# xiph/theora

Measured on AMD Instinct MI355X. Metric: decode frames/sec (4k 4:2:0, bit-exact), higher is better.
Workload: dtype i16; 1 GPU; 4k (3840x2160 coded) 4:2:0, 4 concurrent streams per GPU, keyframe interval 64, content class 'dense', levels form (seeded fragment command streams resident in HBM), loop filter on (flimit 2); streams_per_gpu=4, frame_pool=6, gt_IC=True, parallelism=stream-sharded x1

## Files before the change

theora_amd/csrc/thip_decode.hip:

```cpp
#include <hip/hip_runtime.h>
#include <stdint.h>
#include <stdio.h>
#include <stdlib.h>
#include <string.h>
#include <time.h>

#include <atomic>
#include <mutex>
#include <vector>

#include "../../include/theora_hip.h"
#include "thip_device.h"
#include "thip_ctx.h"
#include "thip_device_guard.h"

using namespace thip;

#define HIP_TRY(expr)                                                                    \
  do {                                                                                   \
    hipError_t e_ = (expr);                                                              \
    if (e_ != hipSuccess) {                                                              \
      fprintf(stderr, "theora_hip: %s failed: %s (%s:%d)\n", #expr, hipGetErrorString(e_), \
              __FILE__, __LINE__);                                                       \
      return THIP_EFAULT;                                                                \
// ... 154 lines not shown
  int64_t frame_serial, out_serial;
  hipEvent_t ev_out2[2];
  int held_img;
  int64_t held_serial;
  int32_t *enq_last_lane;
  int enq_ncoded, enq_nuncoded, enq_nslots, enq_frame_type, enq_flimit, enq_active, enq_last_tile;
  int enq_lf_y0[3], enq_lf_y1[3], enq_lf_any;
  FrameExtras extras;
  int16_t *d_dc;
  uint4 *d_dc_ent;
  uint8_t *d_dc_rowhas;
  uint32_t *fault;
  struct {
    int valid;
    thip_frame_desc d;
    int ring[3];
    FrameExtras extras;
    int64_t serial;
    uint32_t launch_id;
  } redo;
  int redo_owned;
  uint8_t *d_edge;
  uint32_t edge_epoch;
  uint8_t *d_edge_sb;
  uint32_t edge_epoch_sb;
  int device_dc, enq_device_dc;
  int16_t *h_dc, *d_dc_in;
  uint8_t *h_flags, *d_flags;
  uint32_t *h_tok, *d_tok;
  uint32_t *h_slot_tok, *d_slot_tok;
  uint16_t *h_dq, *d_dq;
  uint16_t *h_dqp, *d_dqp;
  size_t tok_cap;
  int tok_ready;
  int enq_ntok, enq_tok_slots, enq_dense_slots;
  int enq_levels_hint;
  int enq_level_slots;
  int enq_tile_blocks;
  uint32_t *h_tl, *d_tl;
  uint32_t *h_tl_buf[2];
  int tl_buf;
  int64_t tl_buf_serial[2];
  size_t tl_cap;
  int tl_ready;
  int16_t *d_tl_tmp;
  uint8_t *d_tl_last;
// ... 381 lines not shown
  DeviceGuard dg(st->device);
  (void)hipDeviceSynchronize();
  if (st->fault) (void)hipHostFree(st->fault);
  for (int b = 0; b < 3; b++)
    if (st->frames[b]) (void)hipFree(st->frames[b]);
  if (st->coded_map) (void)hipFree(st->coded_map);
  if (st->h_info) (void)hipHostFree(st->h_info);
  if (st->h_coeffs) (void)hipHostFree(st->h_coeffs);
  if (st->h_slot0) (void)hipHostFree(st->h_slot0);
  for (int b = 0; b < 2; b++)
    if (st->h_out[b]) (void)hipHostFree(st->h_out[b]);
  for (int k = 0; k < 2; k++)
    if (st->ev_out2[k]) (void)hipEventDestroy(st->ev_out2[k]);
  if (st->ev_staging) (void)hipEventDestroy(st->ev_staging);
  if (st->d_info) (void)hipFree(st->d_info);
  if (st->d_coeffs) (void)hipFree(st->d_coeffs);
  if (st->d_slot0) (void)hipFree(st->d_slot0);
  if (st->d_dc) (void)hipFree(st->d_dc);
  if (st->d_dc_ent) (void)hipFree(st->d_dc_ent);
  if (st->d_dc_rowhas) (void)hipFree(st->d_dc_rowhas);
  if (st->ev_order) (void)hipEventDestroy(st->ev_order);
  if (st->d_edge) (void)hipFree(st->d_edge);
  if (st->d_edge_sb) (void)hipFree(st->d_edge_sb);
  for (int k = 0; k < 2; k++)
    if (st->h_tl_buf[k]) (void)hipHostFree(st->h_tl_buf[k]);
  if (st->d_tl) (void)hipFree(st->d_tl);
  if (st->d_tl_tmp) (void)hipFree(st->d_tl_tmp);
  if (st->d_tl_last) (void)hipFree(st->d_tl_last);
  if (st->d_tl_slot) (void)hipFree(st->d_tl_slot);
  if (st->d_tl_arr) (void)hipFree(st->d_tl_arr);
  if (st->d_tl_pos) (void)hipFree(st->d_tl_pos);
  if (st->d_tl_wide) (void)hipFree(st->d_tl_wide);
  if (st->d_tl_rank) (void)hipFree(st->d_tl_rank);
  if (st->d_frag_pos) (void)hipFree(st->d_frag_pos);
  if (st->pp_frame) (void)hipFree(st->pp_frame);
  if (st->pp_var) (void)hipFree(st->pp_var);
  if (st->pp_qis) (void)hipFree(st->pp_qis);
  if (st->pp_done) (void)hipFree(st->pp_done);
  if (st->h_pp_qis) (void)hipHostFree(st->h_pp_qis);
  if (st->ev_pp) (void)hipEventDestroy(st->ev_pp);
  if (st->d_dc_in) (void)hipFree(st->d_dc_in);
  if (st->h_dc) (void)hipHostFree(st->h_dc);
  if (st->h_flags) (void)hipHostFree(st->h_flags);
  if (st->h_tok) (void)hipHostFree(st->h_tok);
  if (st->h_slot_tok) (void)hipHostFree(st->h_slot_tok);
  if (st->h_dq) (void)hipHostFree(st->h_dq);
// ... 500 lines not shown
  if (fits && !dc_global) {
    HIP_TRY(set_dynamic_lds(reinterpret_cast<const void *>(k_dc_wave), kDcwLdsMax, 3));
    hipLaunchKernelGGL(k_dc_prepare, dim3(max_rows, 3, ndc), dim3((max_nh + 63) & ~63), 0, s, D);
    hipLaunchKernelGGL(k_dc_wave, dim3(3, ndc), dim3(64), (size_t)lds, s, D);
  } else {
    hipLaunchKernelGGL(k_dc_unpredict, dim3(3, ndc), dim3((max_rows + 63) & ~63), 0, s, D);
  }
  HIP_TRY(hipGetLastError());
  return THIP_OK;
}

static int take_edge_records(thip_state *st, StreamK &K, uint8_t **buf, uint32_t *epoch, size_t bytes, uint32_t tag, hipStream_t s) {
  if (!*buf) {
    HIP_TRY(hipMalloc((void **)buf, bytes));
    HIP_TRY(hipMemsetAsync(*buf, 0, bytes, s));
  }
  K.edge = *buf;
  *epoch = *epoch % 4095u + 1u;
  K.epoch = *epoch;
  st->redo.launch_id = K.epoch | tag;
  return THIP_OK;
}

static int launch_recon(Chunk &C, thip_state *const *states, bool levels, bool two_passes, hipStream_t s) {
  const BatchK &B = C.B;
  const int nlive = C.nlive;
  const int fuse = two_passes ? 0 : THIP_OPT("fuse");
  if (fuse == 3 && C.any_lf && !C.any_skip && xcd_round_robin(states[C.live[0]]->device)) {
    int longest = 1, total_tiles = 0;
    for (int j = 0; j < nlive; j++) total_tiles += B.s[j].tile_end[2];
    const int sb_tiles = THIP_OPT("sb_tiles");
    const bool small = sb_tiles > 0 && total_tiles < sb_tiles;
    for (int j = 0; j < nlive; j++) {
      thip_state *st = states[C.live[j]];
      StreamK &K = C.B.s[j];
      if (st->tiles.tiles_y[0] > 4096) return THIP_EIMPL;
      longest = std::max(longest, fill_bands(K, st));
      const int rc = small ? take_edge_records(st, K, &st->d_edge_sb, &st->edge_epoch_sb, (size_t)4 * K.tile_end[2] * Tf4::kRec, 0x1000u, s)
                           : take_edge_records(st, K, &st->d_edge, &st->edge_epoch, (size_t)K.tile_end[2] * kTfRec, 0u, s);
      if (rc < 0) return rc;
    }
    ScopedTimer t(s, THIP_KERNEL_RECON);
    if (small) {
      if (levels) hipLaunchKernelGGL(k_recon_lf_sb<true>, dim3(8 * longest, nlive), dim3(256), 0, s, B);
      else hipLaunchKernelGGL(k_recon_lf_sb<false>, dim3(8 * longest, nlive), dim3(256), 0, s, B);
    } else if (levels) hipLaunchKernelGGL(k_recon_lf<true>, dim3(8 * longest, nlive), dim3(64), 0, s, B);
    else hipLaunchKernelGGL(k_recon_lf<false>, dim3(8 * longest, nlive), dim3(64), 0, s, B);
  } else {
    {
      ScopedTimer t(s, THIP_KERNEL_RECON);
      if (levels) hipLaunchKernelGGL(k_recon<true>, dim3(C.max_wg, nlive), dim3(64 * THIP_RECON_WG_WAVES), 0, s, B);
      else hipLaunchKernelGGL(k_recon<false>, dim3(C.max_wg, nlive), dim3(64 * THIP_RECON_WG_WAVES), 0, s, B);
    }
    if (C.any_lf) {
      ScopedTimer t(s, THIP_KERNEL_LOOPFILTER);
      hipLaunchKernelGGL(k_loopfilter, dim3(C.max_seam_wg, nlive), dim3(THIP_LF_WG), 0, s, B);
    }
  }
  HIP_TRY(hipGetLastError());
  return THIP_OK;
}

static int advance_rings(const Chunk &C, thip_state *const *states, const thip_frame_desc *descs, hipStream_t s) {
// ... 1527 lines not shown
```

theora_amd/csrc/thip_fused.h:

```cpp
#pragma once

#ifndef THIP_TF_PITCH
#define THIP_TF_PITCH 144
#endif
template <int BW>
struct TfGeom {
  static constexpr int kBW = BW;
  static constexpr int kPitch = BW == 16 ? THIP_TF_PITCH : 8 * BW + 16;
  static constexpr int kX0 = 8;
  static constexpr int kImgRows = 40;
  static constexpr int kFlagOff = kImgRows * kPitch;
  static constexpr int kFlagPitch = BW + 4;
  static constexpr int kRowDwords = 2 * BW;
  static constexpr int kBotUnits = (2 * kRowDwords + 2) / 3, kRightUnits = 11;
  static constexpr int kBot = 0;
  static constexpr int kRight = kBotUnits * 16;
  static constexpr int kTop = (kBotUnits + kRightUnits) * 16;
  static constexpr int kRec = ((2 * kBotUnits + kRightUnits) * 16 + 127) & ~127;
};
typedef TfGeom<16> Tf16;
constexpr int kTfPitch = Tf16::kPitch, kTfX0 = Tf16::kX0, kTfImgRows = Tf16::kImgRows, kTfFlagOff = Tf16::kFlagOff, kTfFlagPitch = Tf16::kFlagPitch;
constexpr int kTfLds = 7168;
static_assert(kTfFlagOff + 6 * kTfFlagPitch <= kTfLds, "the image lives in the wave's staging area");
static_assert(kLdsTabOff + 768 <= kTfLds && kLdsTabOff >= 6 * 1024, "the tables sit behind six staged pieces");
constexpr int kTfUnit = 16;
constexpr int kTfBotUnits = Tf16::kBotUnits, kTfRightUnits = Tf16::kRightUnits;
constexpr int kTfBot = Tf16::kBot, kTfRight = Tf16::kRight, kTfTop = Tf16::kTop, kTfRec = Tf16::kRec;
static_assert(kTfBotUnits == 22 && kTfRight == 352 && kTfTop == 528 && kTfRec == 896, "the record layout of rounds 3 and 4");

typedef uint32_t tf_u32x4 __attribute__((ext_vector_type(4)));
__device__ __forceinline__ void tf_store_unit(uint8_t *p, uint4 v, bool through) {
  if (through) {
    const tf_u32x4 w = {v.x, v.y, v.z, v.w};
    asm volatile("global_store_dwordx4 %0, %1, off sc0 sc1" ::"v"(p), "v"(w) : "memory");
  } else {
    *reinterpret_cast<uint4 *>(p) = v;
  }
}
__device__ __forceinline__ uint4 tf_load_unit(const uint8_t *p) {
  tf_u32x4 w;
  asm volatile("global_load_dwordx4 %0, %1, off sc0 sc1\n\ts_waitcnt vmcnt(0)" : "=&v"(w) : "v"(p) : "memory");
  return make_uint4(w.x, w.y, w.z, w.w);
}

template <class G>
__device__ __forceinline__ int tf_rows_at(int idx, int ri0) { return (ri0 + idx / G::kRowDwords) * G::kPitch + G::kX0 + (idx % G::kRowDwords) * 4; }
template <class G>
// ... 188 lines not shown
#ifdef THIP_PRIO_SEQ
#define THIP_PRIO_AT(i) __builtin_amdgcn_s_setprio((THIP_PRIO_SEQ >> (12 - 4 * (i))) & 3)
#else
#define THIP_PRIO_AT(i) do { } while (0)
#endif
#ifndef THIP_TF_WAVES_PER_EU
#define THIP_TF_WAVES_PER_EU 5
#endif
template <bool LEVELS>
__global__ __launch_bounds__(64, THIP_TF_WAVES_PER_EU) void k_recon_lf(const BatchK B) {
  __shared__ uint4 s_tf[kTfLds / 16];
  const StreamK &S = B.s[blockIdx.y];
  const int lane = (int)threadIdx.x & 63;
  const int band = (int)blockIdx.x & 7, jb = (int)blockIdx.x >> 3;
  const uint2 *info_p = S.info;
  const int4 *coeffs_p = S.coeffs;
  const uint32_t *slot0_p = S.tile_slot0;
  uint8_t *self = S.self;
  const uint8_t *prev = S.prev, *gold = S.gold;
  uint8_t *coded_map = S.coded_map;
  const int16_t *dc_p = S.dc;
  const uint4 *dq_p = S.dequant;
  uint8_t *edge_p = S.edge;
  const int te0 = S.tile_end[0], te1 = S.tile_end[1];
  const int sqpx = S.qpx, sqpy = S.qpy;
  const int L2 = (S.debug & 256) ? 0 : S.flimit2;
  const bool poison = (S.debug & 512) != 0;
  const bool cell_general = (S.debug & 1024) != 0;
  const int max_spins = poison ? 256 : (1 << 20);
  uint32_t *fault_p = S.fault;
  const uint32_t ep = S.epoch;
  const int bu0 = S.band_u0[band], bu1 = S.band_u0[band + 1];
  asm volatile("" ::"s"(info_p), "s"(coeffs_p), "s"(slot0_p), "s"(self), "s"(prev), "s"(gold), "s"(coded_map), "s"(dc_p), "s"(dq_p), "s"(edge_p),
               "s"(te0), "s"(te1), "s"(sqpx), "s"(sqpy), "s"(L2), "s"(ep), "s"(bu0), "s"(bu1), "s"(fault_p));
  const int u = bu0 + jb;
  if (u >= bu1) return;
  const int pli = (u >= te0 ? 1 : 0) + (u >= te1 ? 1 : 0);
  const int rel = u - (pli == 0 ? 0 : (pli == 1 ? te0 : te1));
  const int tiles_x = S.spec_tx[pli];
  const int sby = rel / tiles_x, t = rel - sby * tiles_x;
  bool spec = false;
  uint32_t spec_slot0 = 0;
  if (LEVELS && S.spec_on) {
    if (sby < S.spec_rows[pli]) {
      spec = true;
      spec_slot0 = S.spec_base[pli] + (uint32_t)(sby * S.spec_rowunits[pli]) + 64u * (uint32_t)t;
      const uint32_t unit = min(spec_slot0 + (uint32_t)lane, S.spec_last);
#pragma unroll
      for (int q = 0; q < 4; q++)
        __builtin_amdgcn_global_load_lds((const __attribute__((address_space(1))) void *)unit_piece(coeffs_p, unit, q),
                                         (__attribute__((address_space(3))) void *)(s_tf + q * 64), 16, 0, THIP_COEF_CPOL);
    }
  }
  [[maybe_unused]] unsigned long long *tr = nullptr;
#ifdef THIP_TRACE
  if (g_trace_buf && lane == 0) {
    tr = g_trace_buf + ((size_t)blockIdx.y * gridDim.x + blockIdx.x) * 12;
    unsigned hwid, xcc;
    asm volatile("s_getreg_b32 %0, hwreg(HW_REG_HW_ID)\n\ts_getreg_b32 %1, hwreg(HW_REG_XCC_ID)" : "=s"(hwid), "=s"(xcc));
    tr[9] = hwid;
    tr[10] = (unsigned long long)xcc | (unsigned long long)u << 8;
  }
#endif
  THIP_TR(tr, 0);
  THIP_PRIO_AT(0);
  constexpr bool levels = LEVELS;
  if (levels) tables_to_lds(dq_p, pli, lane, s_tf);
  const PlaneK G = S.pl[pli];
  const int fy0 = S.lf_y0[pli], fy1 = S.lf_y1[pli];
  asm volatile("" ::"s"(G.nh), "s"(G.nv), "s"(G.stride), "s"(G.off), "s"(G.tiles_x), "s"(G.tiles_y), "s"(G.fro), "s"(fy0), "s"(fy1));
  const int nh = G.nh, nv = G.nv;
  const bool has_left = t > 0, row_end = t == tiles_x - 1;
  const bool has_up = sby > 0, has_dn = sby < G.tiles_y - 1;
  const bool up_in = has_up && u - tiles_x >= bu0, dn_in = has_dn && u + tiles_x < bu1;
  const bool xb_up = has_up && !up_in;
  const bool xb_dn = has_dn && !dn_in;

  const int hh = lane & 15;
  const int lx = (lane >> 4) * 4 + hilb_col(hh), ly = hilb_row(hh);
  const int bx = t * 16 + lx, by = sby * 4 + ly;
  const bool valid = bx < nh && by < nv;
  const uint32_t slot0w = slot0_p[u];
  const uint2 info = info_p[(size_t)u * THIP_TILE_FRAGS + lane];
  uint32_t dcv = 0;
  if (dc_p) dcv = 0x10000u | (uint16_t)dc_p[G.fro + min(by, nv - 1) * nh + min(bx, nh - 1)];
  asm volatile("" ::"s"(slot0w), "v"(info.x), "v"(dcv));
#ifdef THIP_TRACE
  THIP_TR(tr, 1);
#endif
  if (levels && !dc_p) dcv = 0x10000u | (info.y & 0xFFFFu);
  const CoefForm F = coef_form(slot0w, levels);
  ReconLane L;
  L.flags = valid ? info.x : 0u;
  L.dcq = info.y >> 16;
  L.dcraw = dcv;
  L.dcp = ((uint32_t)(((int)(int16_t)((dcv ? dcv : info.y) & 0xFFFFu) * (int)L.dcq + 15) >> 5) & 0xFFFFu) * 0x00010001u;
  L.coded = (L.flags & THIP_INFO_CODED) != 0;
  L.dc_only = L.coded && (L.flags & THIP_INFO_DC_ONLY) != 0;
  L.has_coeff = L.coded && !L.dc_only;
  L.x0 = bx * 8;
  L.y0 = by * 8;
  const bool own_all_coded = __all(valid && L.coded);
  ReconPlane R;
  R.self = self + G.off;
  R.prev = prev + G.off;
  R.gold = gold + G.off;
  R.coded_map = coded_map + G.fro;
  R.nh = nh;
  R.nv = nv;
  R.stride = G.stride;
  R.qpx = pli != 0 && sqpx;
  R.qpy = pli != 0 && sqpy;
  R.debug = 0;
  R.tr = nullptr;
  uint8_t *const lds = reinterpret_cast<uint8_t *>(s_tf);
  uint32_t *const lds_dw = reinterpret_cast<uint32_t *>(s_tf);
  uint32_t *const meta = lds_dw + 1024;

  const uint64_t mask = __ballot(L.has_coeff);
  const int nown = __popcll(mask);
  const uint32_t prefix = __builtin_amdgcn_mbcnt_hi((uint32_t)(mask >> 32), __builtin_amdgcn_mbcnt_lo((uint32_t)mask, 0u));
  PredWin Q;
  Q.border = false;
  bool inter = false;
  const uint8_t *ref = nullptr;
  const uint32_t fill = L.dc_only ? L.dcp : 0u;
  uint32_t Y[32];
  if (nown == 0) {
    if (valid) recon_issue<true>(R, L, Q, inter, ref);
    THIP_PRIO_AT(1);
  } else if (nown <= 16) {
    int4 Wc[1][2];
    residual_shared_load<4>(coeffs_p, F, nown, lane, Wc);
    if (valid) recon_issue<true>(R, L, Q, inter, ref);
    THIP_PRIO_AT(1);
    residual_shared<4>(Wc, F, lds_dw, meta, lane, L, prefix, Y);
  } else if (nown <= 32) {
    int4 Wc[2][2];
    residual_shared_load<2>(coeffs_p, F, nown, lane, Wc);
    if (valid) recon_issue<true>(R, L, Q, inter, ref);
    THIP_PRIO_AT(1);
    residual_shared<2, true>(Wc, F, lds_dw, meta, lane, L, prefix, Y);
  } else {
    int4 w7 = make_int4(0, 0, 0, 0);
    const bool spec_hit = spec && nown == 64 && !F.wide && F.slot0 == spec_slot0;
    if (!spec_hit) dense_issue<7>(coeffs_p, F, L.has_coeff, prefix, s_tf, w7);
    if (valid) recon_issue<true>(R, L, Q, inter, ref);
    THIP_PRIO_AT(1);
    if (!spec_hit) asm volatile("s_waitcnt vmcnt(0)" ::: "memory");
    dense_finish<7>(coeffs_p, F, L.has_coeff, prefix, s_tf, lane, L, w7, Y);
  }
  if (!L.has_coeff) {
#pragma unroll
    for (int i = 0; i < 32; i++) Y[i] = fill;
  }
#ifdef THIP_TRACE
  asm volatile("" : "+v"(Y[0]), "+v"(Y[31]));
  THIP_TR(tr, 11);
#endif
  uint2 rows[8];
  recon_rows<true>(R, Q, inter, Y, rows, L.coded ? L.flags : 0u, L.x0);
#ifdef THIP_TRACE
  asm volatile("" : "+v"(rows[0].x), "+v"(rows[7].y));
  THIP_TR(tr, 2);
#endif

  THIP_PRIO_AT(2);
  uint8_t *const myrec = edge_p + (size_t)u * kTfRec;
  const uint8_t *const rec_up = myrec - (ptrdiff_t)tiles_x * kTfRec, *const rec_left = myrec - kTfRec;
  const uint8_t *const rec_ul = rec_up - kTfRec;
  const bool need_ul = up_in && has_left;
  lds_settle();
  if (valid) {
    uint8_t *img = lds + (ly * 8 + 4) * kTfPitch + kTfX0 + lx * 8;
#pragma unroll
    for (int r = 0; r < 8; r++) *reinterpret_cast<uint2 *>(img + r * kTfPitch) = rows[r];
  }
  lds[kTfFlagOff + (ly + 1) * kTfFlagPitch + lx + 1] = (valid && L.coded) ? 1 : 0;
  lds_settle();
  {
    const int fi = lane < 16 ? 4 * kTfFlagPitch + lane + 1
                             : (lane < 20 ? (lane - 16 + 1) * kTfFlagPitch + 16 : (lane >= 32 && lane < 48 ? kTfFlagPitch + (lane - 32) + 1 : 0));
    uint64_t fm = 0x0000FFFF000FFFFFull;
    if (!flags_lazy || !own_all_coded) {
// ... 31 lines not shown
    } else if (lane < kTfBotUnits + kTfRightUnits) {
#pragma unroll
      for (int j = 0; j < 3; j++) {
        const int idx = 3 * (lane - kTfBotUnits) + j;
        if (idx < 32) *reinterpret_cast<uint32_t *>(lds + tf_col_at<Tf16>(idx, 4, -4)) = d[j];
      }
    } else if (lane == kTfBotUnits + kTfRightUnits) {
#pragma unroll
      for (int j = 0; j < 2; j++) *reinterpret_cast<uint32_t *>(lds + tf_col_at<Tf16>(2 + j, 0, -4)) = d[j];
    }
    w_up = (uint32_t)__builtin_amdgcn_readlane((int)un.w, 0);
    w_left = (uint32_t)__builtin_amdgcn_readlane((int)un.w, kTfBotUnits);
    w_ul = (uint32_t)__builtin_amdgcn_readlane((int)un.w, kTfBotUnits + kTfRightUnits);
    nb_all_coded = (!up_in || (w_up & 0xFFFFu) == 0xFFFFu) && (!has_left || (w_left & 0xF0000u) == 0xF0000u) && (!need_ul || (w_ul & 0x80000u) != 0);
#ifndef THIP_NO_CELL_FAST
    cells_coded = own_all_coded && nb_all_coded && L2 != 0 && !cell_general && fy0 <= 4 * sby - (up_in ? 1 : 0) && fy1 >= 4 * sby + 4;
#endif
    if (!flags_lazy || !cells_coded) tf_neighbour_flags(lds, lane, w_up, w_left, w_ul);
    lds_settle();
    THIP_TR(tr, 6);
  }

  THIP_PRIO_AT(3);
  const int top_lo = has_up ? (xb_up ? 6 : 2) : 0;
  const uint32_t top_mask = xb_up ? 96u : 0xFFu;
  {
    const int m = lane >> 4;
#ifndef THIP_NO_CELL_FAST
    const bool coded = cells_coded;
    if (coded && has_left && up_in)
      tf_cell_all_coded<Tf16, false>(lds, R.self, R.stride, t, sby, lane & 15, m, L2, 2, false);
#ifndef THIP_NO_CELL_EDGE
    else if (coded)
      tf_cell_all_coded<Tf16, true>(lds, R.self, R.stride, t, sby, lane & 15, m, L2, has_up ? (xb_up ? 6 : 2) : 4, !has_left);
#endif
    else
#endif
      tf_cell<Tf16>(lds, R.self, R.stride, nh, nv, t, sby, lane & 15, m, true, L2, fy0, fy1, m == 0 ? top_lo : 0, 8, m == 0 ? top_mask : 0xFFu, m == 3);
  }
  THIP_TR(tr, 7);

  const bool extra_col = row_end && (nh & 15) == 0;
  const bool extra_row = xb_dn || (!has_dn && (nv & 3) == 0);
  if (extra_col || extra_row) {
    [[maybe_unused]] bool dn_all_coded = true;
    uint32_t w_dn = 0, w_dl = 0;
    if (xb_dn) {
      const uint8_t *const rec_dn = myrec + (ptrdiff_t)tiles_x * kTfRec, *const rec_dl = rec_dn - kTfRec;
      const uint8_t *src = nullptr;
      if (lane < kTfBotUnits) src = rec_dn + kTfTop + lane * kTfUnit;
      else if (lane == kTfBotUnits && has_left) src = rec_dl + kTfRight;
      const uint4 un = tf_fetch_unit(src, ep, fault_p, max_spins, ep);
      const uint32_t d[3] = {un.x, un.y, un.z};
      if (lane < kTfBotUnits) {
#pragma unroll
        for (int j = 0; j < 3; j++) {
          const int idx = 3 * lane + j;
          if (idx < 64) *reinterpret_cast<uint32_t *>(lds + tf_rows_at<Tf16>(idx, 36)) = d[j];
        }
      } else if (lane == kTfBotUnits) {
#pragma unroll
        for (int j = 0; j < 2; j++) *reinterpret_cast<uint32_t *>(lds + tf_col_at<Tf16>(j, 36, -4)) = d[j];
      }
      w_dn = (uint32_t)__builtin_amdgcn_readlane((int)un.w, 0);
      w_dl = (uint32_t)__builtin_amdgcn_readlane((int)un.w, kTfBotUnits);
      dn_all_coded = (w_dn & 0xFFFFu) == 0xFFFFu && (!has_left || (w_dl & 0x10000u) != 0);
// ... 30 lines not shown
```

theora_amd/csrc/thip_kernels.h:

```cpp
#pragma once
#include <hip/hip_runtime.h>
#include <stdint.h>

#include "../../include/theora_hip.h"
#include "thip_device.h"

using namespace thip;

constexpr uint32_t kHilbRow = 0u | 0u << 2 | 1u << 4 | 1u << 6 | 2u << 8 | 3u << 10 | 3u << 12 | 2u << 14 |
                              2u << 16 | 3u << 18 | 3u << 20 | 2u << 22 | 1u << 24 | 1u << 26 | 0u << 28 | 0u << 30;
constexpr uint32_t kHilbCol = 0u | 1u << 2 | 1u << 4 | 0u << 6 | 0u << 8 | 0u << 10 | 1u << 12 | 1u << 14 |
                              2u << 16 | 2u << 18 | 3u << 20 | 3u << 22 | 3u << 24 | 2u << 26 | 2u << 28 | 3u << 30;
constexpr uint64_t kHilbInv = 0ull | 1ull << 4 | 14ull << 8 | 15ull << 12 |
                              3ull << 16 | 2ull << 20 | 13ull << 24 | 12ull << 28 |
                              4ull << 32 | 7ull << 36 | 8ull << 40 | 11ull << 44 |
                              5ull << 48 | 6ull << 52 | 9ull << 56 | 10ull << 60;

__host__ __device__ inline int hilb_row(int h) { return (int)((kHilbRow >> (2 * h)) & 3u); }
__host__ __device__ inline int hilb_col(int h) { return (int)((kHilbCol >> (2 * h)) & 3u); }
__host__ __device__ inline int hilb_inv(int r, int c) { return (int)((kHilbInv >> (4 * (r * 4 + c))) & 15ull); }

struct PlaneK {
  int nh, nv;
  int stride;
  int off;
  int tiles_x;
  int tile_off;
  int fro;
  float rcp_cx;
  int tiles_y;
};

struct StreamK {
  const uint2 *info;
  const int4 *coeffs;
  const uint32_t *tile_slot0;
  uint8_t *self;
  const uint8_t *prev;
  const uint8_t *gold;
  uint8_t *coded_map;
  const uint8_t *coded_prev;
  const int16_t *dc;
  const uint4 *dequant;
  int skip_ok;
  int flimit2;
  int qpx, qpy;
  int tile_end[3];
  int cell_end[3];
  int lf_y0[3], lf_y1[3];
  int debug;
  int lf_sparse;
  uint8_t *edge;
  uint32_t epoch;
  int band_u0[9];
  uint32_t *fault;
  int spec_on;
// ... 159 lines not shown
  }
}

__device__ __forceinline__ void load_slot(const int4 *coeffs, uint32_t slot, uint32_t P[32]) {
  const int4 *tp = coeffs + ((size_t)(slot >> 6) * 512 + (slot & 63));
#pragma unroll
  for (int q = 0; q < 8; q++) {
    const int4 w = tp[q * 64];
    P[q * 4 + 0] = (uint32_t)w.x;
    P[q * 4 + 1] = (uint32_t)w.y;
    P[q * 4 + 2] = (uint32_t)w.z;
    P[q * 4 + 3] = (uint32_t)w.w;
  }
}

struct PredWin {
  Row12 w[9];
  int sx, sy, mx2, my2;
  bool border;
};

__device__ __forceinline__ int pred_xw(int xs, int W) { return max(min(xs, W - 12), 0) & ~3; }

template <bool INFRAME = false>
__device__ __forceinline__ void pred_issue(PredWin &Q, const uint8_t *prev, const uint8_t *gold, bool use_prev, int stride, int W, int H, int x0,
                                           int y0, uint32_t flags, bool qpx, bool qpy) {
  const int dx = (int)(int8_t)(flags >> THIP_INFO_MVX_SHIFT);
  const int dy = (int)(int8_t)(flags >> THIP_INFO_MVY_SHIFT);
  int mx, my;
  mv_axis(dx, qpx, mx, Q.mx2);
  mv_axis(dy, qpy, my, Q.my2);
  Q.sx = x0 + mx;
  Q.sy = y0 + my;
  const int xs = Q.sx + min(Q.mx2, 0), ys = Q.sy + min(Q.my2, 0);
  Q.border = ((int)(xs < 0) | (int)(Q.sx + max(Q.mx2, 0) + 8 > W) | (int)(ys < 0) | (int)(Q.sy + max(Q.my2, 0) + 8 > H)) != 0;
#ifndef THIP_NO_PRED_INFRAME
  if (INFRAME) {
    const bool all_prev = __all(use_prev);
    if ((all_prev || !__any(use_prev)) && !__any(Q.border)) {
      const BufRsrc plane = buf_rsrc(all_prev ? prev : gold, (uint32_t)(H * stride));
      const uint32_t o0 = (uint32_t)(ys * stride + pred_xw(xs, W));
#pragma unroll
      for (int r = 0; r < 8; r++) Q.w[r] = load_row12(plane, o0, r * stride);
      Q.w[8] = load_row12(plane, o0 + (Q.my2 != 0 ? (uint32_t)stride : 0u), 7 * stride);
      return;
    }
  }
#endif
  const uint8_t *p1 = (use_prev ? prev : gold) + pred_xw(xs, W);
#pragma unroll
  for (int r = 0; r < 9; r++) {
    const int y = min(max(ys + (r < 8 ? r : (Q.my2 != 0 ? 8 : 7)), 0), H - 1);
    Q.w[r] = load_row12(p1 + (ptrdiff_t)y * stride);
  }
}

__device__ __forceinline__ void pred_sel(int col0, int xw, int W, uint32_t &sel, bool &k) {
  int c[4];
#pragma unroll
  for (int i = 0; i < 4; i++) c[i] = min(max(col0 + i, 0), W - 1) - xw;
  k = c[0] >= 4;
  const int o = k ? 4 : 0;
  sel = (uint32_t)(c[0] - o) | (uint32_t)(c[1] - o) << 8 | (uint32_t)(c[2] - o) << 16 | (uint32_t)(c[3] - o) << 24;
}
__device__ __forceinline__ uint32_t pred_pick(const Row12 &w, uint32_t sel, bool k) {
  return __builtin_amdgcn_perm(k ? w.c : w.b, k ? w.b : w.a, sel);
}

__device__ __forceinline__ void pred_finish(const PredWin &Qin, int W, uint2 pred[8], uint32_t flags, int x0, bool qpx, bool qpy) {
#ifndef THIP_NO_PRED_REMAT
  PredWin Q;
  {
    asm volatile("" : "+v"(flags), "+v"(x0));
    const int dx = (int)(int8_t)(flags >> THIP_INFO_MVX_SHIFT), dy = (int)(int8_t)(flags >> THIP_INFO_MVY_SHIFT);
    int mx, my;
    mv_axis(dx, qpx, mx, Q.mx2);
    mv_axis(dy, qpy, my, Q.my2);
    Q.sx = x0 + mx;
    Q.border = Qin.border;
#pragma unroll
    for (int r = 0; r < 9; r++) Q.w[r] = Qin.w[r];
  }
#else
  const PredWin &Q = Qin;
#endif
  const int xw = pred_xw(Q.sx + min(Q.mx2, 0), W);
  const bool ra = Q.my2 < 0, rb = Q.my2 > 0;
  const bool two = (Q.mx2 | Q.my2) != 0;
  if (!__any(Q.border)) {
    const int offA = Q.sx - xw, offB = Q.sx + Q.mx2 - xw;
    const uint32_t selT = extract_sel(ra ? offB : offA), selU = extract_sel(ra ? offA : offB);
    const bool down = Q.my2 != 0;
#pragma unroll
    for (int r = 0; r < 8; r++) pred[r] = extract8s(Q.w[r], selT);
    if (two) {
      uint2 u = extract8s(Q.w[0], selU);
#pragma unroll
      for (int r = 0; r < 8; r++) {
        const uint2 n = extract8s(Q.w[r + 1], selU);
        pred[r].x = avg4_trunc(pred[r].x, down ? n.x : u.x);
        pred[r].y = avg4_trunc(pred[r].y, down ? n.y : u.y);
        u = n;
      }
    }
  } else {
    uint32_t sa0, sa1, sb0, sb1;
    bool ka0, ka1, kb0, kb1;
    pred_sel(Q.sx, xw, W, sa0, ka0);
    pred_sel(Q.sx + 4, xw, W, sa1, ka1);
    pred_sel(Q.sx + Q.mx2, xw, W, sb0, kb0);
    pred_sel(Q.sx + Q.mx2 + 4, xw, W, sb1, kb1);
#pragma unroll
    for (int r = 0; r < 8; r++) {
      const Row12 wa = ra ? Q.w[r + 1] : Q.w[r];
      pred[r] = make_uint2(pred_pick(wa, sa0, ka0), pred_pick(wa, sa1, ka1));
      if (two) {
        const Row12 wb = rb ? Q.w[r + 1] : Q.w[r];
        pred[r].x = avg4_trunc(pred[r].x, pred_pick(wb, sb0, kb0));
        pred[r].y = avg4_trunc(pred[r].y, pred_pick(wb, sb1, kb1));
      }
    }
  }
}

#ifndef THIP_RECON_WAVES
#ifndef THIP_COEF_CPOL
#define THIP_COEF_CPOL 0
#endif
#define THIP_RECON_WAVES 4
#endif
#ifndef THIP_RECON_WG_WAVES
#define THIP_RECON_WG_WAVES 1
#endif

#ifdef THIP_TRACE
__device__ unsigned long long *g_trace_buf;
__device__ __forceinline__ unsigned long long trace_now() {
  unsigned long long t;
  asm volatile("s_memrealtime %0\n\ts_waitcnt lgkmcnt(0)" : "=s"(t)::"memory");
  return t;
// ... 53 lines not shown
  asm("v_mul_lo_u16_sdwa %0, sext(%1), %2 dst_sel:WORD_0 dst_unused:UNUSED_PAD src0_sel:BYTE_0 src1_sel:WORD_0" : "=v"(even) : "v"(w), "v"(t_even));
  asm("v_mul_lo_u16_sdwa %0, sext(%1), %2 dst_sel:WORD_1 dst_unused:UNUSED_PRESERVE src0_sel:BYTE_2 src1_sel:WORD_1" : "+v"(even) : "v"(w), "v"(t_even));
  asm("v_mul_lo_u16_sdwa %0, sext(%1), %2 dst_sel:WORD_0 dst_unused:UNUSED_PAD src0_sel:BYTE_1 src1_sel:WORD_0" : "=v"(odd) : "v"(w), "v"(t_odd));
  asm("v_mul_lo_u16_sdwa %0, sext(%1), %2 dst_sel:WORD_1 dst_unused:UNUSED_PRESERVE src0_sel:BYTE_3 src1_sel:WORD_1" : "+v"(odd) : "v"(w), "v"(t_odd));
}
#else
__device__ __forceinline__ void dequant_levels(uint32_t w, uint32_t t_even, uint32_t t_odd, uint32_t &even, uint32_t &odd) {
  uint32_t e, o;
  unpack_levels(w, e, o);
  even = as_u32(as_pk(e) * as_pk(t_even));
  odd = as_u32(as_pk(o) * as_pk(t_odd));
}
#endif
__device__ __forceinline__ uint32_t pk_mul_lo(uint32_t a, uint32_t b) { return as_u32(as_pk(a) * as_pk(b)); }
__device__ __forceinline__ uint32_t table_of(uint32_t flags) {
  return ((flags >> THIP_INFO_QII_SHIFT) & 3u) * 2u + (((flags >> THIP_INFO_REFI_SHIFT) & 3u) != (uint32_t)THIP_FRAME_SELF ? 1u : 0u);
}
__device__ __forceinline__ void tables_to_lds(const uint4 *dequant, int pli, int lane, uint4 *lds_wave, int tab16 = kLdsTabOff / 16) {
  if (lane < 48)
    __builtin_amdgcn_global_load_lds((const __attribute__((address_space(1))) void *)(dequant + pli * 48 + lane),
                                     (__attribute__((address_space(3))) void *)(lds_wave + tab16), 16, 0, 0);
}

template <bool INFRAME = false>
__device__ __forceinline__ void recon_issue(const ReconPlane &R, const ReconLane &L, PredWin &Q, bool &inter,
                                            const uint8_t *&ref, bool write_map = true) {
  const int refi = L.coded ? (int)((L.flags >> THIP_INFO_REFI_SHIFT) & 3u) : THIP_FRAME_PREV;
  inter = refi != THIP_FRAME_SELF && !(R.debug & 2);
  ref = refi == THIP_FRAME_PREV ? R.prev : R.gold;
  Q.border = false;
  if (inter) pred_issue<INFRAME>(Q, R.prev, R.gold, refi == THIP_FRAME_PREV, R.stride, R.nh * 8, R.nv * 8, L.x0, L.y0, L.coded ? L.flags : 0u, R.qpx, R.qpy);
  if (write_map) R.coded_map[(L.y0 >> 3) * R.nh + (L.x0 >> 3)] = L.coded ? 1 : 0;
}

template <bool INTRA_LATE = false>
__device__ __forceinline__ void recon_rows(const ReconPlane &R, const PredWin &Q, bool inter, const uint32_t Y[32],
                                           uint2 rows[8], uint32_t Lflags, int Lx0) {
  uint2 pred[8];
#ifdef THIP_NO_PRED_INFRAME
  constexpr bool late = false;
#else
  constexpr bool late = INTRA_LATE;
#endif
  if (!late) {
#pragma unroll
    for (int r = 0; r < 8; r++) pred[r] = make_uint2(0x80808080u, 0x80808080u);
  }
  if (inter) pred_finish(Q, R.nh * 8, pred, Lflags, Lx0, R.qpx, R.qpy);
  if (late && !__all(inter)) {
    if (!inter) {
#pragma unroll
      for (int r = 0; r < 8; r++) pred[r] = make_uint2(0x80808080u, 0x80808080u);
    }
  }
#pragma unroll
  for (int r = 0; r < 8; r++)
    rows[r] = pk_recon_row(as_pk(Y[r * 4 + 0]), as_pk(Y[r * 4 + 1]), as_pk(Y[r * 4 + 2]), as_pk(Y[r * 4 + 3]), pred[r]);
}

__device__ __forceinline__ void recon_finish(const ReconPlane &R, const ReconLane &L, const PredWin &Q, bool inter,
                                             const uint32_t Y[32]) {
  uint8_t *dst = R.self + (ptrdiff_t)L.y0 * R.stride + L.x0;
  uint2 rows[8];
  recon_rows(R, Q, inter, Y, rows, L.coded ? L.flags : 0u, L.x0);
  if (!(R.debug & 4)) {
#pragma unroll
    for (int r = 0; r < 8; r++) store_row8(dst + (ptrdiff_t)r * R.stride, rows[r]);
  }
}

template <int NLDS>
// ... 594 lines not shown
```

Baseline: 95540 frames/s.

## Precompute per-tile records on host and park MV selectors in LDS

Result: faster. 96610 frames/s (median of 5 runs) (+1.1%).

```diff
diff --git a/theora_amd/csrc/thip_decode.hip b/theora_amd/csrc/thip_decode.hip
--- a/theora_amd/csrc/thip_decode.hip
+++ b/theora_amd/csrc/thip_decode.hip
@@ -200,6 +200,9 @@
   int redo_owned;
   uint8_t *d_edge;
   uint32_t edge_epoch;
+  TileRec *d_tile_rec;
+  TileRec *h_tile_rec;
+  int tile_rec_bands[9];
   uint8_t *d_edge_sb;
   uint32_t edge_epoch_sb;
   int device_dc, enq_device_dc;
@@ -627,6 +630,8 @@
   if (st->ev_order) (void)hipEventDestroy(st->ev_order);
   if (st->d_edge) (void)hipFree(st->d_edge);
   if (st->d_edge_sb) (void)hipFree(st->d_edge_sb);
+  if (st->d_tile_rec) (void)hipFree(st->d_tile_rec);
+  free(st->h_tile_rec);
   for (int k = 0; k < 2; k++)
     if (st->h_tl_buf[k]) (void)hipHostFree(st->h_tl_buf[k]);
   if (st->d_tl) (void)hipFree(st->d_tl);
@@ -1173,6 +1178,59 @@
   return THIP_OK;
 }
 
+static void tile_records(TileRec *out, const StreamK &K) {
+  int u = 0;
+  uint32_t unit0 = 0;
+  for (int pli = 0; pli < 3; pli++) {
+    const PlaneK &G = K.pl[pli];
+    const int tiles_x = G.tiles_x, tiles_y = G.tiles_y;
+    for (int sby = 0; sby < tiles_y; sby++)
+      for (int t = 0; t < tiles_x; t++, u++) {
+        int band = 0;
+        while (band < 7 && u >= K.band_u0[band + 1]) band++;
+        const int bu0 = K.band_u0[band], bu1 = K.band_u0[band + 1];
+        const bool has_left = t > 0, row_end = t == tiles_x - 1;
+        const bool has_up = sby > 0, has_dn = sby < tiles_y - 1;
+        const bool up_in = has_up && u - tiles_x >= bu0, dn_in = has_dn && u + tiles_x < bu1;
+        const bool xb_up = has_up && !up_in, xb_dn = has_dn && !dn_in;
+        const bool extra_col = row_end && (G.nh & 15) == 0;
+        const bool extra_row = xb_dn || (!has_dn && (G.nv & 3) == 0);
+        const int top_lo = has_up ? (xb_up ? 6 : 2) : 0;
+        const bool spec = sby < G.nv / 4;
+        TileRec &T = out[u];
+        memset(&T, 0, sizeof(T));
+        T.bits = (uint32_t)pli | (has_left ? kTrHasLeft : 0u) | (row_end ? kTrRowEnd : 0u) | (has_up ? kTrHasUp : 0u) | (has_dn ? kTrHasDn : 0u) |
+                 (up_in ? kTrUpIn : 0u) | (dn_in ? kTrDnIn : 0u) | (extra_col ? kTrExtraCol : 0u) | (extra_row ? kTrExtraRow : 0u) |
+                 (spec ? kTrSpec : 0u) | (uint32_t)top_lo << kTrTopLoShift | (uint32_t)tiles_x << kTrTilesXShift;
+        T.place = (uint32_t)t | (uint32_t)sby << 16;
+        T.spec0 = unit0 + (uint32_t)sby * 4u * (uint32_t)G.nh + 64u * (uint32_t)t;
+        T.nh = G.nh;
+        T.nv = G.nv;
+        T.stride = G.stride;
+        T.off = G.off;
+        T.fro = G.fro;
+      }
+    unit0 += (uint32_t)G.nh * (uint32_t)G.nv;
+  }
+}
+static int take_tile_records(thip_state *st, StreamK &K, hipStream_t s) {
+  const size_t bytes = sizeof(TileRec) * (size_t)K.tile_end[2];
+  const bool fresh = !st->d_tile_rec;
+  if (fresh) {
+    if (!st->h_tile_rec) st->h_tile_rec = (TileRec *)malloc(bytes);
+    if (!st->h_tile_rec) return THIP_EFAULT;
+    HIP_TRY(hipMalloc((void **)&st->d_tile_rec, bytes));
+  }
+  if (fresh || memcmp(st->tile_rec_bands, K.band_u0, sizeof(st->tile_rec_bands)) != 0) {
+    if (!fresh) HIP_TRY(hipDeviceSynchronize());
+    tile_records(st->h_tile_rec, K);
+    memcpy(st->tile_rec_bands, K.band_u0, sizeof(st->tile_rec_bands));
+    HIP_TRY(hipMemcpyAsync(st->d_tile_rec, st->h_tile_rec, bytes, hipMemcpyHostToDevice, s));
+  }
+  K.tile_rec = st->d_tile_rec;
+  return THIP_OK;
+}
+
 static int launch_recon(Chunk &C, thip_state *const *states, bool levels, bool two_passes, hipStream_t s) {
   const BatchK &B = C.B;
   const int nlive = C.nlive;
@@ -1190,6 +1248,10 @@
       const int rc = small ? take_edge_records(st, K, &st->d_edge_sb, &st->edge_epoch_sb, (size_t)4 * K.tile_end[2] * Tf4::kRec, 0x1000u, s)
                            : take_edge_records(st, K, &st->d_edge, &st->edge_epoch, (size_t)K.tile_end[2] * kTfRec, 0u, s);
       if (rc < 0) return rc;
+      if (!small) {
+        const int trc = take_tile_records(st, K, s);
+        if (trc < 0) return trc;
+      }
     }
     ScopedTimer t(s, THIP_KERNEL_RECON);
     if (small) {
diff --git a/theora_amd/csrc/thip_fused.h b/theora_amd/csrc/thip_fused.h
--- a/theora_amd/csrc/thip_fused.h
+++ b/theora_amd/csrc/thip_fused.h
@@ -23,6 +23,13 @@
 constexpr int kTfLds = 7168;
 static_assert(kTfFlagOff + 6 * kTfFlagPitch <= kTfLds, "the image lives in the wave's staging area");
 static_assert(kLdsTabOff + 768 <= kTfLds && kLdsTabOff >= 6 * 1024, "the tables sit behind six staged pieces");
+constexpr int kTfParkOff = kLdsTabOff + 768;
+static_assert(kTfParkOff + 64 * 4 == kTfLds, "one parked dword per lane behind the tables");
+#ifdef THIP_NO_MV_ONCE
+constexpr bool kTfMvOnce = false;
+#else
+constexpr bool kTfMvOnce = true;
+#endif
 constexpr int kTfUnit = 16;
 constexpr int kTfBotUnits = Tf16::kBotUnits, kTfRightUnits = Tf16::kRightUnits;
 constexpr int kTfBot = Tf16::kBot, kTfRight = Tf16::kRight, kTfTop = Tf16::kTop, kTfRec = Tf16::kRec;
@@ -257,7 +264,9 @@
   const int16_t *dc_p = S.dc;
   const uint4 *dq_p = S.dequant;
   uint8_t *edge_p = S.edge;
+#ifdef THIP_NO_TILE_REC
   const int te0 = S.tile_end[0], te1 = S.tile_end[1];
+#endif
   const int sqpx = S.qpx, sqpy = S.qpy;
   const int L2 = (S.debug & 256) ? 0 : S.flimit2;
   const bool poison = (S.debug & 512) != 0;
@@ -266,6 +275,46 @@
   uint32_t *fault_p = S.fault;
   const uint32_t ep = S.epoch;
   const int bu0 = S.band_u0[band], bu1 = S.band_u0[band + 1];
+#ifndef THIP_NO_TILE_REC
+  const TileRec *rec_p = S.tile_rec;
+  const int spec_on = S.spec_on;
+  const uint32_t spec_last = S.spec_last;
+  const int fy0_0 = S.lf_y0[0], fy0_1 = S.lf_y0[1], fy0_2 = S.lf_y0[2], fy1_0 = S.lf_y1[0], fy1_1 = S.lf_y1[1], fy1_2 = S.lf_y1[2];
+  asm volatile("" ::"s"(info_p), "s"(coeffs_p), "s"(slot0_p), "s"(self), "s"(prev), "s"(gold), "s"(coded_map), "s"(dc_p), "s"(dq_p), "s"(edge_p),
+               "s"(rec_p), "s"(spec_on), "s"(spec_last), "s"(sqpx), "s"(sqpy), "s"(L2), "s"(ep), "s"(bu0), "s"(bu1), "s"(fault_p),
+               "s"(fy0_0), "s"(fy0_1), "s"(fy0_2), "s"(fy1_0), "s"(fy1_1), "s"(fy1_2));
+  const int u = bu0 + jb;
+  if (u >= bu1) return;
+  TileRec T;
+  {
+    typedef uint32_t tr_u32x8 __attribute__((ext_vector_type(8)));
+    const tr_u32x8 rw = *(const __attribute__((address_space(4))) tr_u32x8 *)(uintptr_t)(rec_p + u);
+    T.bits = rw[0];
+    T.place = rw[1];
+    T.spec0 = rw[2];
+    T.nh = (int)rw[3];
+    T.nv = (int)rw[4];
+    T.stride = (int)rw[5];
+    T.off = (int)rw[6];
+    T.fro = (int)rw[7];
+  }
+  const int pli = (int)(T.bits & 3u);
+  const int tiles_x = (int)(T.bits >> kTrTilesXShift);
+  const int t = (int)(T.place & 0xFFFFu), sby = (int)(T.place >> 16);
+  bool spec = false;
+  uint32_t spec_slot0 = 0;
+  if (LEVELS && spec_on) {
+    if (T.bits & kTrSpec) {
+      spec = true;
+      spec_slot0 = T.spec0;
+      const uint32_t unit = min(spec_slot0 + (uint32_t)lane, spec_last);
+#pragma unroll
+      for (int q = 0; q < 4; q++)
+        __builtin_amdgcn_global_load_lds((const __attribute__((address_space(1))) void *)unit_piece(coeffs_p, unit, q),
+                                         (__attribute__((address_space(3))) void *)(s_tf + q * 64), 16, 0, THIP_COEF_CPOL);
+    }
+  }
+#else
   asm volatile("" ::"s"(info_p), "s"(coeffs_p), "s"(slot0_p), "s"(self), "s"(prev), "s"(gold), "s"(coded_map), "s"(dc_p), "s"(dq_p), "s"(edge_p),
                "s"(te0), "s"(te1), "s"(sqpx), "s"(sqpy), "s"(L2), "s"(ep), "s"(bu0), "s"(bu1), "s"(fault_p));
   const int u = bu0 + jb;
@@ -287,6 +336,7 @@
                                          (__attribute__((address_space(3))) void *)(s_tf + q * 64), 16, 0, THIP_COEF_CPOL);
     }
   }
+#endif
   [[maybe_unused]] unsigned long long *tr = nullptr;
 #ifdef THIP_TRACE
   if (g_trace_buf && lane == 0) {
@@ -301,6 +351,14 @@
   THIP_PRIO_AT(0);
   constexpr bool levels = LEVELS;
   if (levels) tables_to_lds(dq_p, pli, lane, s_tf);
+#ifndef THIP_NO_TILE_REC
+  struct { int nh, nv, stride, off, fro; } G = {T.nh, T.nv, T.stride, T.off, T.fro};
+  const int fy0 = pli == 0 ? fy0_0 : (pli == 1 ? fy0_1 : fy0_2), fy1 = pli == 0 ? fy1_0 : (pli == 1 ? fy1_1 : fy1_2);
+  const int nh = G.nh, nv = G.nv;
+  const bool has_left = (T.bits & kTrHasLeft) != 0;
+  const bool has_up = (T.bits & kTrHasUp) != 0, has_dn = (T.bits & kTrHasDn) != 0;
+  const bool up_in = (T.bits & kTrUpIn) != 0, dn_in = (T.bits & kTrDnIn) != 0;
+#else
   const PlaneK G = S.pl[pli];
   const int fy0 = S.lf_y0[pli], fy1 = S.lf_y1[pli];
   asm volatile("" ::"s"(G.nh), "s"(G.nv), "s"(G.stride), "s"(G.off), "s"(G.tiles_x), "s"(G.tiles_y), "s"(G.fro), "s"(fy0), "s"(fy1));
@@ -308,6 +366,7 @@
   const bool has_left = t > 0, row_end = t == tiles_x - 1;
   const bool has_up = sby > 0, has_dn = sby < G.tiles_y - 1;
   const bool up_in = has_up && u - tiles_x >= bu0, dn_in = has_dn && u + tiles_x < bu1;
+#endif
   const bool xb_up = has_up && !up_in;
   const bool xb_dn = has_dn && !dn_in;
 
@@ -351,6 +410,8 @@
   uint8_t *const lds = reinterpret_cast<uint8_t *>(s_tf);
   uint32_t *const lds_dw = reinterpret_cast<uint32_t *>(s_tf);
   uint32_t *const meta = lds_dw + 1024;
+  constexpr bool park_mv = LEVELS && kTfMvOnce;
+  uint32_t *const park = lds_dw + kTfParkOff / 4 + lane;
 
   const uint64_t mask = __ballot(L.has_coeff);
   const int nown = __popcll(mask);
@@ -362,25 +423,25 @@
   const uint32_t fill = L.dc_only ? L.dcp : 0u;
   uint32_t Y[32];
   if (nown == 0) {
-    if (valid) recon_issue<true>(R, L, Q, inter, ref);
+    if (valid) recon_issue<true, park_mv>(R, L, Q, inter, ref, true, park);
     THIP_PRIO_AT(1);
   } else if (nown <= 16) {
     int4 Wc[1][2];
     residual_shared_load<4>(coeffs_p, F, nown, lane, Wc);
-    if (valid) recon_issue<true>(R, L, Q, inter, ref);
+    if (valid) recon_issue<true, park_mv>(R, L, Q, inter, ref, true, park);
     THIP_PRIO_AT(1);
     residual_shared<4>(Wc, F, lds_dw, meta, lane, L, prefix, Y);
   } else if (nown <= 32) {
     int4 Wc[2][2];
     residual_shared_load<2>(coeffs_p, F, nown, lane, Wc);
-    if (valid) recon_issue<true>(R, L, Q, inter, ref);
+    if (valid) recon_issue<true, park_mv>(R, L, Q, inter, ref, true, park);
     THIP_PRIO_AT(1);
     residual_shared<2, true>(Wc, F, lds_dw, meta, lane, L, prefix, Y);
   } else {
     int4 w7 = make_int4(0, 0, 0, 0);
     const bool spec_hit = spec && nown == 64 && !F.wide && F.slot0 == spec_slot0;
     if (!spec_hit) dense_issue<7>(coeffs_p, F, L.has_coeff, prefix, s_tf, w7);
-    if (valid) recon_issue<true>(R, L, Q, inter, ref);
+    if (valid) recon_issue<true, park_mv>(R, L, Q, inter, ref, true, park);
     THIP_PRIO_AT(1);
     if (!spec_hit) asm volatile("s_waitcnt vmcnt(0)" ::: "memory");
     dense_finish<7>(coeffs_p, F, L.has_coeff, prefix, s_tf, lane, L, w7, Y);
@@ -394,7 +455,7 @@
   THIP_TR(tr, 11);
 #endif
   uint2 rows[8];
-  recon_rows<true>(R, Q, inter, Y, rows, L.coded ? L.flags : 0u, L.x0);
+  recon_rows<true, park_mv>(R, Q, inter, Y, rows, L.coded ? L.flags : 0u, L.x0, park);
 #ifdef THIP_TRACE
   asm volatile("" : "+v"(rows[0].x), "+v"(rows[7].y));
   THIP_TR(tr, 2);
@@ -472,7 +533,11 @@
   }
 
   THIP_PRIO_AT(3);
+#ifndef THIP_NO_TILE_REC
+  const int top_lo = (int)(T.bits >> kTrTopLoShift) & 15;
+#else
   const int top_lo = has_up ? (xb_up ? 6 : 2) : 0;
+#endif
   const uint32_t top_mask = xb_up ? 96u : 0xFFu;
   {
     const int m = lane >> 4;
@@ -490,8 +555,12 @@
   }
   THIP_TR(tr, 7);
 
+#ifndef THIP_NO_TILE_REC
+  const bool extra_col = (T.bits & kTrExtraCol) != 0, extra_row = (T.bits & kTrExtraRow) != 0;
+#else
   const bool extra_col = row_end && (nh & 15) == 0;
   const bool extra_row = xb_dn || (!has_dn && (nv & 3) == 0);
+#endif
   if (extra_col || extra_row) {
     [[maybe_unused]] bool dn_all_coded = true;
     uint32_t w_dn = 0, w_dl = 0;
diff --git a/theora_amd/csrc/thip_kernels.h b/theora_amd/csrc/thip_kernels.h
--- a/theora_amd/csrc/thip_kernels.h
+++ b/theora_amd/csrc/thip_kernels.h
@@ -31,7 +31,19 @@
   int tiles_y;
 };
 
+struct TileRec {
+  uint32_t bits;
+  uint32_t place;
+  uint32_t spec0;
+  int nh, nv, stride, off, fro;
+};
+static_assert(sizeof(TileRec) == 32, "one scalar load of eight dwords");
+constexpr uint32_t kTrHasLeft = 1u << 2, kTrRowEnd = 1u << 3, kTrHasUp = 1u << 4, kTrHasDn = 1u << 5, kTrUpIn = 1u << 6, kTrDnIn = 1u << 7,
+                   kTrExtraCol = 1u << 8, kTrExtraRow = 1u << 9, kTrSpec = 1u << 10;
+constexpr int kTrTopLoShift = 12, kTrTilesXShift = 16;
+
 struct StreamK {
+  const TileRec *tile_rec;
   const uint2 *info;
   const int4 *coeffs;
   const uint32_t *tile_slot0;
@@ -237,9 +249,19 @@
 
 __device__ __forceinline__ int pred_xw(int xs, int W) { return max(min(xs, W - 12), 0) & ~3; }
 
-template <bool INFRAME = false>
+constexpr uint32_t kParkDown = 1u << 16, kParkTwo = 3u << 16, kParkBorder = 1u << 31;
+__device__ __forceinline__ uint32_t pred_park(const PredWin &Q, int xw) {
+  const uint32_t offA = (uint32_t)(Q.sx - xw), offB = offA + (uint32_t)Q.mx2;
+  const bool ra = Q.my2 < 0;
+  uint32_t w = (ra ? offB : offA) | (ra ? offA : offB) << 8;
+  w |= ((uint32_t)Q.my2 & 1u) << 16;
+  w |= ((uint32_t)Q.mx2 & 1u) << 17;
+  return w | (Q.border ? kParkBorder : 0u);
+}
+
+template <bool INFRAME = false, bool PARK = false>
 __device__ __forceinline__ void pred_issue(PredWin &Q, const uint8_t *prev, const uint8_t *gold, bool use_prev, int stride, int W, int H, int x0,
-                                           int y0, uint32_t flags, bool qpx, bool qpy) {
+                                           int y0, uint32_t flags, bool qpx, bool qpy, uint32_t *park = nullptr) {
   const int dx = (int)(int8_t)(flags >> THIP_INFO_MVX_SHIFT);
   const int dy = (int)(int8_t)(flags >> THIP_INFO_MVY_SHIFT);
   int mx, my;
@@ -249,6 +271,7 @@
   Q.sy = y0 + my;
   const int xs = Q.sx + min(Q.mx2, 0), ys = Q.sy + min(Q.my2, 0);
   Q.border = ((int)(xs < 0) | (int)(Q.sx + max(Q.mx2, 0) + 8 > W) | (int)(ys < 0) | (int)(Q.sy + max(Q.my2, 0) + 8 > H)) != 0;
+  if (PARK) *park = pred_park(Q, pred_xw(xs, W));
 #ifndef THIP_NO_PRED_INFRAME
   if (INFRAME) {
     const bool all_prev = __all(use_prev);
@@ -282,55 +305,80 @@
   return __builtin_amdgcn_perm(k ? w.c : w.b, k ? w.b : w.a, sel);
 }
 
-__device__ __forceinline__ void pred_finish(const PredWin &Qin, int W, uint2 pred[8], uint32_t flags, int x0, bool qpx, bool qpy) {
+template <bool PARK = false>
+__device__ __forceinline__ void pred_finish(const PredWin &Qin, int W, uint2 pred[8], uint32_t flags, int x0, bool qpx, bool qpy,
+                                            const uint32_t *park = nullptr) {
+  uint32_t pw = 0;
+  if (PARK) pw = *park;
 #ifndef THIP_NO_PRED_REMAT
-  PredWin Q;
-  {
-    asm volatile("" : "+v"(flags), "+v"(x0));
-    const int dx = (int)(int8_t)(flags >> THIP_INFO_MVX_SHIFT), dy = (int)(int8_t)(flags >> THIP_INFO_MVY_SHIFT);
-    int mx, my;
-    mv_axis(dx, qpx, mx, Q.mx2);
-    mv_axis(dy, qpy, my, Q.my2);
-    Q.sx = x0 + mx;
-    Q.border = Qin.border;
-#pragma unroll
-    for (int r = 0; r < 9; r++) Q.w[r] = Qin.w[r];
-  }
+  constexpr bool remat = true;
 #else
-  const PredWin &Q = Qin;
-#endif
-  const int xw = pred_xw(Q.sx + min(Q.mx2, 0), W);
-  const bool ra = Q.my2 < 0, rb = Q.my2 > 0;
-  const bool two = (Q.mx2 | Q.my2) != 0;
-  if (!__any(Q.border)) {
-    const int offA = Q.sx - xw, offB = Q.sx + Q.mx2 - xw;
-    const uint32_t selT = extract_sel(ra ? offB : offA), selU = extract_sel(ra ? offA : offB);
-    const bool down = Q.my2 != 0;
-#pragma unroll
-    for (int r = 0; r < 8; r++) pred[r] = extract8s(Q.w[r], selT);
+  constexpr bool remat = false;
+#endif
+  const bool border = PARK ? (int)pw < 0 : Qin.border;
+  if (!__any(border)) {
+    uint32_t selT, selU;
+    bool down, two;
+    if (PARK) {
+      selT = 0x03020100u + __builtin_amdgcn_perm(pw, pw, 0x00000000u);
+      selU = 0x03020100u + __builtin_amdgcn_perm(pw, pw, 0x01010101u);
+      down = (pw & kParkDown) != 0;
+      two = (pw & kParkTwo) != 0;
+    } else {
+      int sx = Qin.sx, mx2 = Qin.mx2, my2 = Qin.my2;
+      if (remat) {
+        asm volatile("" : "+v"(flags), "+v"(x0));
+        const int dx = (int)(int8_t)(flags >> THIP_INFO_MVX_SHIFT), dy = (int)(int8_t)(flags >> THIP_INFO_MVY_SHIFT);
+        int mx, my;
+        mv_axis(dx, qpx, mx, mx2);
+        mv_axis(dy, qpy, my, my2);
+        sx = x0 + mx;
+      }
+      const int xw = pred_xw(sx + min(mx2, 0), W);
+      const bool ra = my2 < 0;
+      const int offA = sx - xw, offB = sx + mx2 - xw;
+      selT = extract_sel(ra ? offB : offA);
+      selU = extract_sel(ra ? offA : offB);
+      down = my2 != 0;
+      two = (mx2 | my2) != 0;
+    }
+#pragma unroll
+    for (int r = 0; r < 8; r++) pred[r] = extract8s(Qin.w[r], selT);
     if (two) {
-      uint2 u = extract8s(Q.w[0], selU);
+      uint2 u = extract8s(Qin.w[0], selU);
 #pragma unroll
       for (int r = 0; r < 8; r++) {
-        const uint2 n = extract8s(Q.w[r + 1], selU);
+        const uint2 n = extract8s(Qin.w[r + 1], selU);
         pred[r].x = avg4_trunc(pred[r].x, down ? n.x : u.x);
         pred[r].y = avg4_trunc(pred[r].y, down ? n.y : u.y);
         u = n;
       }
     }
   } else {
+    int sx = Qin.sx, mx2 = Qin.mx2, my2 = Qin.my2;
+    if (remat || PARK) {
+      asm volatile("" : "+v"(flags), "+v"(x0));
+      const int dx = (int)(int8_t)(flags >> THIP_INFO_MVX_SHIFT), dy = (int)(int8_t)(flags >> THIP_INFO_MVY_SHIFT);
+      int mx, my;
+      mv_axis(dx, qpx, mx, mx2);
+      mv_axis(dy, qpy, my, my2);
+      sx = x0 + mx;
+    }
+    const int xw = pred_xw(sx + min(mx2, 0), W);
+    const bool ra = my2 < 0, rb = my2 > 0;
+    const bool two = (mx2 | my2) != 0;
     uint32_t sa0, sa1, sb0, sb1;
     bool ka0, ka1, kb0, kb1;
-    pred_sel(Q.sx, xw, W, sa0, ka0);
-    pred_sel(Q.sx + 4, xw, W, sa1, ka1);
-    pred_sel(Q.sx + Q.mx2, xw, W, sb0, kb0);
-    pred_sel(Q.sx + Q.mx2 + 4, xw, W, sb1, kb1);
+    pred_sel(sx, xw, W, sa0, ka0);
+    pred_sel(sx + 4, xw, W, sa1, ka1);
+    pred_sel(sx + mx2, xw, W, sb0, kb0);
+    pred_sel(sx + mx2 + 4, xw, W, sb1, kb1);
 #pragma unroll
     for (int r = 0; r < 8; r++) {
-      const Row12 wa = ra ? Q.w[r + 1] : Q.w[r];
+      const Row12 wa = ra ? Qin.w[r + 1] : Qin.w[r];
       pred[r] = make_uint2(pred_pick(wa, sa0, ka0), pred_pick(wa, sa1, ka1));
       if (two) {
-        const Row12 wb = rb ? Q.w[r + 1] : Q.w[r];
+        const Row12 wb = rb ? Qin.w[r + 1] : Qin.w[r];
         pred[r].x = avg4_trunc(pred[r].x, pred_pick(wb, sb0, kb0));
         pred[r].y = avg4_trunc(pred[r].y, pred_pick(wb, sb1, kb1));
       }
@@ -430,20 +478,20 @@
                                      (__attribute__((address_space(3))) void *)(lds_wave + tab16), 16, 0, 0);
 }
 
-template <bool INFRAME = false>
+template <bool INFRAME = false, bool PARK = false>
 __device__ __forceinline__ void recon_issue(const ReconPlane &R, const ReconLane &L, PredWin &Q, bool &inter,
-                                            const uint8_t *&ref, bool write_map = true) {
+                                            const uint8_t *&ref, bool write_map = true, uint32_t *park = nullptr) {
   const int refi = L.coded ? (int)((L.flags >> THIP_INFO_REFI_SHIFT) & 3u) : THIP_FRAME_PREV;
   inter = refi != THIP_FRAME_SELF && !(R.debug & 2);
   ref = refi == THIP_FRAME_PREV ? R.prev : R.gold;
   Q.border = false;
-  if (inter) pred_issue<INFRAME>(Q, R.prev, R.gold, refi == THIP_FRAME_PREV, R.stride, R.nh * 8, R.nv * 8, L.x0, L.y0, L.coded ? L.flags : 0u, R.qpx, R.qpy);
+  if (inter) pred_issue<INFRAME, PARK>(Q, R.prev, R.gold, refi == THIP_FRAME_PREV, R.stride, R.nh * 8, R.nv * 8, L.x0, L.y0, L.coded ? L.flags : 0u, R.qpx, R.qpy, park);
   if (write_map) R.coded_map[(L.y0 >> 3) * R.nh + (L.x0 >> 3)] = L.coded ? 1 : 0;
 }
 
-template <bool INTRA_LATE = false>
+template <bool INTRA_LATE = false, bool PARK = false>
 __device__ __forceinline__ void recon_rows(const ReconPlane &R, const PredWin &Q, bool inter, const uint32_t Y[32],
-                                           uint2 rows[8], uint32_t Lflags, int Lx0) {
+                                           uint2 rows[8], uint32_t Lflags, int Lx0, const uint32_t *park = nullptr) {
   uint2 pred[8];
 #ifdef THIP_NO_PRED_INFRAME
   constexpr bool late = false;
@@ -454,7 +502,7 @@
 #pragma unroll
     for (int r = 0; r < 8; r++) pred[r] = make_uint2(0x80808080u, 0x80808080u);
   }
-  if (inter) pred_finish(Q, R.nh * 8, pred, Lflags, Lx0, R.qpx, R.qpy);
+  if (inter) pred_finish<PARK>(Q, R.nh * 8, pred, Lflags, Lx0, R.qpx, R.qpy, park);
   if (late && !__all(inter)) {
     if (!inter) {
 #pragma unroll
```
